# arpitbansal297/Cold-Diffusion-Models

Measured on AMD Instinct MI355X. Metric: unet_train_imgs_per_sec, higher is better.
Workload: dtype f32 storage/accumulate; dense-conv GEMM operands bf16x3; 1 GPU; CelebA-128 denoising cold diffusion (BASELINE config 3): Unet(dim=64,(1,2,4,8),ch=3) @128x128, T=200, optimizer step = 2 micro-batches x 32 img (one fused forward / backward pass over all of them: same draws, same gradient sum) + Adam + EMA/10; per_gpu_batch=32, gradient_accumulate_every=2, parallelism=single

## Files before the change

cold-diffusion-models_amd/csrc/k_conv_rowhalo.hip:

```cpp
#include "cdf_conv_sp.h"

template <int W, int BN, int NS = 3, int NCH = 2, int BM = 256>
__global__ void __launch_bounds__(512, 1) conv_igemm_rowhalo_stream_kernel(SpxArgs a) {
    constexpr int WM = BM / 64, WN = 8 / WM, NW = 8, BK = 32, RE = CDF_SP_RE, MT = BM / WM / 32, NB = 3;
    static_assert(BM == 256 && WM * WN == 8 && MT == 2, "8 waves (4 x 2) of 64-row tiles");
    static_assert(NCH % 2 == 0, "an even number of tap-row groups per tile returns the pipeline to row buffer 0");
    using L = RowHaloLayout<W, BN, BM>;
    using Segs = typename L::Segs;
    constexpr int EROWS = L::EROWS, CP = L::CP;
    constexpr int TH = L::TH, HW2 = L::HW2, RH = L::RH;
    constexpr int TAG = Segs::PER_WAVE;
    constexpr int NT = BN / WN / 32;
    constexpr int SB = BN / 16 / NW;
    static_assert(SB * NW * 16 == BN || BN == 64, "B tile must split into 16-row segments");
    constexpr int SBI = BN == 64 ? 1 : SB;
    constexpr int PLANE_A = L::PLANE_A, PLANE_B = L::PLANE_B;
    CDF_DYN_SMEM(smem_raw);
    unsigned short* smem = (unsigned short*)smem_raw;
    float* const cs = (float*)(smem + L::OFF_CS);

    const int tid = threadIdx.x, lane = tid & 63, wave = __builtin_amdgcn_readfirstlane(tid >> 6);
    const int wm = wave / WN, wn = wave % WN;
    const int M = a.B * a.QH * a.QW;
    const int tiles_n = (a.Cout + BN - 1) / BN, tiles_m = M / BM, ntiles = tiles_m * tiles_n;
    const CdfPhase& ph = a.ph[0];
    const int tpi = a.H / TH;

    const int srow = cdf_dma_row(lane), q8 = cdf_dma_col(lane);
    int a_seg[TAG], a_ry[TAG], a_x[TAG];
#pragma unroll
    for (int q = 0; q < TAG; ++q) {
        const int g = a_seg[q] = Segs::seg(wave, q);
        const int r = g * 16 + srow;
        a_ry[q] = r < RH ? r / HW2 : -(1 << 20);
        a_x[q] = r - (r / HW2) * HW2 - 1;
    }
    auto fetch_a = [&](int img, int y0, int c, int dy, int buf) {
        unsigned short* base = smem + L::a_off(buf);
#pragma unroll
        for (int q = 0; q < TAG; ++q) {
            const int y = y0 + a_ry[q] + dy;
            const bool ok = img >= 0 && (unsigned)y < (unsigned)a.H && (unsigned)a_x[q] < (unsigned)W;
            const size_t off = ((size_t)(((ok ? img : 0) * a.H + (ok ? y : 0)) * W + (ok ? a_x[q] : 0))) * (unsigned)a.ldx + (unsigned)(c * BK + q8);
            unsigned short* seg = base + a_seg[q] * 16 * RE;
            CDF_GLDS16_K(ok ? a.x_hi + off : a.zero, seg);
            if constexpr (NS == 3) CDF_GLDS16_K(ok ? a.x_lo + off : a.zero, seg + PLANE_A);
        }
    };
    auto fetch_b = [&](int tile_n, int c, int wi, int stage) {
        unsigned short* st = smem + L::b_off(stage);
#pragma unroll
        for (int p = 0; p < SBI; ++p) {
            const int seg = BN == 64 ? (wave & 3) : wave * SB + p;
            const size_t woff = cdf_w_off(wi, a.Cout, cdf_w_row(tile_n * BN + seg * 16 + srow, a.Cout), a.ldk, c * BK + q8);
            CDF_GLDS16_K(a.w_hi + woff, st + seg * 16 * RE);
            if constexpr (NS == 3) CDF_GLDS16_K(a.w_lo + woff, st + PLANE_B + seg * 16 * RE);
        }
    };
    constexpr int NPL = NS == 3 ? 2 : 1;
    constexpr int PB = NPL * SBI, PAG = NPL * TAG;

    const int half = lane >> 5, l31 = lane & 31;
    int row0[MT];
#pragma unroll
    for (int i = 0; i < MT; ++i) {
        const int pix = wm * (BM / WM) + i * 32 + l31;
        const int py = pix / W, px = pix - py * W;
        row0[i] = py * HW2 + px + 1;
    }
    const bool late = a.dephase != 0 && wave >= NW / 2;

    auto tile_pos = [&](int v, int& img, int& y0, int& tn, int& tm) {
        if (v < ntiles) {
            const int tile = cdf_xcd_order(v, ntiles);
            tm = tile / tiles_n;
            tn = tile - tm * tiles_n;
            img = tm / tpi;
            y0 = (tm - img * tpi) * TH;
        } else {
            img = -1; y0 = 0; tn = 0; tm = 0;
        }
    };
    int img, y0, tile_n, tile_m;
    int v = blockIdx.x;
    tile_pos(v, img, y0, tile_n, tile_m);
    const bool fast_epi = cdf_epi_tile_ok<BM, BN>(a, M) && cdf_epi_family_ok(a.epi, NS == 1);
    fetch_a(img, y0, 0, ph.dy[0], 0);
    fetch_b(tile_n, 0, ph.wi[0], 0);
    fetch_b(tile_n, 0, ph.wi[1], 1);
    CDF_WAIT_DMA_LEAVE(PB);
    CDF_LDS_BARRIER();

    while (img >= 0) {
        int img_n, y0_n, tile_n_n, tile_m_n;
        tile_pos(v + gridDim.x, img_n, y0_n, tile_n_n, tile_m_n);
        f32x16_t acc[MT][NT];
        cdf_acc_zero(acc);
        bf16x8_v ah[2][MT], al[2][MT], bh[2][NT], bl[2][NT];
        if (late) cdf_frag_zero(ah, al, bh, bl);
        auto mma_frags = [&]() { cdf_mma_tile<NS, MT, NT>(acc, ah, al, bh, bl); };
        int row0t[MT], l31t = l31;
#pragma unroll
        for (int i = 0; i < MT; ++i) row0t[i] = row0[i];
#ifndef CDF_EMU
#pragma unroll
        for (int i = 0; i < MT; ++i) asm volatile("" : "+v"(row0t[i]));
        asm volatile("" : "+v"(l31t));
#endif
        const int swbt = (l31t >> 2) & 3;
#pragma unroll
        for (int g = 0; g < 3; ++g) {
#pragma unroll
            for (int c = 0; c < NCH; ++c) {
#pragma unroll
                for (int i3 = 0; i3 < 3; ++i3) {
                    const int t = 3 * g + i3;
                    const int step = (g * NCH + c) * 3 + i3;
                    const int par = (g * NCH + c) & 1, rd = step % NB;
                    {
                        const int s2 = step + 2, gc2 = (s2 / 3) % (3 * NCH);
                        const bool over = s2 >= 9 * NCH;
                        const int g2 = gc2 / NCH, c2 = gc2 - g2 * NCH;
                        fetch_b(over ? tile_n_n : tile_n, c2, ph.wi[3 * g2 + s2 % 3], s2 % NB);
                    }
                    if (i3 == 0) {
                        const bool lastc = c + 1 == NCH, over = lastc && g == 2;
                        const int nc = lastc ? 0 : c + 1, ng = over ? 0 : (lastc ? g + 1 : g);
                        fetch_a(over ? img_n : img, over ? y0_n : y0, nc, ph.dy[3 * ng], par ^ 1);
                    }
                    int sa_e = L::a_off(par), sb_e = L::b_off(rd);
#ifndef CDF_EMU
                    asm volatile("" : "+s"(sa_e), "+s"(sb_e));
#endif
                    const unsigned short* sa = smem + sa_e;
                    const unsigned short* sb = smem + sb_e;
                    const int dx = ph.dx[t];
                    auto read_frags = [&]() {
#pragma unroll
                        for (int ks = 0; ks < 2; ++ks) {
                            cdf_read_frags_halo<NS, PLANE_A>(ah[ks], al[ks], sa, ks, half, row0t, dx);
                            cdf_read_frags<NS, PLANE_B>(bh[ks], bl[ks], sb, ks, half, wn * (BN / WN) + l31t, swbt);
                        }
                    };
                    cdf_dephased_step(late, read_frags, mma_frags);
                    if (i3 <= 1)
                        CDF_WAIT_DMA_LEAVE(PB + PAG);
                    else
                        CDF_WAIT_DMA_LEAVE(PB);
                    CDF_LDS_BARRIER();
                }
            }
        }
        if (late) mma_frags();
        auto dump = [&](int hp) {
            if ((wm * 64) / EROWS == hp) {
                int base = (wm * 64 - hp * EROWS + 4 * half) * CP + wn * (BN / WN) + l31;
#ifndef CDF_EMU
                asm volatile("" : "+v"(base));
#endif
                cdf_acc_stage(cs + base, CP, 0, 0, acc, 0, 0);
            }
        };
        if (fast_epi) {
            const long long trow = (long long)tile_m * BM;
            cdf_epi_dispatch<NS == 1>(a.epi, [&](auto spec) {
                using E = cdf_epi_fast<BN, EROWS, 512, decltype(spec)>;
                f32x4_t q[E::NR], bs[2];
                cdf_epi_load_bias<BN, 512>(a, bs, trow, tile_n * BN, tid);
                E::load(a, q, trow, tile_n * BN, tid);
                dump(0);
                CDF_LDS_BARRIER();
                E::template finish<true>(a, q, bs, cs, trow, tile_n * BN, tid, trow + EROWS);
                CDF_LDS_BARRIER();
                dump(1);
                CDF_LDS_BARRIER();
                E::template finish<false>(a, q, bs, cs, trow + EROWS, tile_n * BN, tid);
                CDF_LDS_BARRIER();
            });
        } else {
#pragma unroll 1
            for (int hp = 0; hp < 2; ++hp) {
                dump(hp);
                CDF_LDS_BARRIER();
                cdf_epilogue_rows<BN, EROWS, 512>(a, ph, a.y, cs, tile_m * BM + hp * EROWS, tile_n * BN, M, tid, [](int p) { return p; });
                CDF_LDS_BARRIER();
            }
        }
        img = img_n; y0 = y0_n; tile_n = tile_n_n; tile_m = tile_m_n;
        v += gridDim.x;
    }
    CDF_WAIT_DMA_LEAVE(0);
}

template <int NS, int W, int BN>
static int launch_igemm_rowhalo_stream(const SpxArgs& a, int M, hipStream_t s, int reserve, CdfPlan* plan) {
    using L = RowHaloLayout<W, BN>;
    const int tiles = (M / 256) * cdf_cdiv(a.Cout, BN);
#ifdef CDF_EMU
    int ncu = cdf_num_cus() - reserve;
    if (ncu < 1) ncu = 1;
#else
    int ncu = cdf_num_cus() - (reserve + 7) / 8 * 8;
    if (ncu < 8) ncu = 8;
#endif
    const int grid = tiles < ncu ? tiles : ncu;
    if (plan) return cdf_plan_set(plan, CDF_FORM_ROWHALO, 256, BN, a.Cin == 64 ? 2 : 4, 1, W, tiles, grid);
    if (a.Cin == 64)
        CDF_LAUNCH_LDS((conv_igemm_rowhalo_stream_kernel<W, BN, NS, 2>), dim3(grid), dim3(512), L::bytes, s, a);
    else
        CDF_LAUNCH_LDS((conv_igemm_rowhalo_stream_kernel<W, BN, NS, 4>), dim3(grid), dim3(512), L::bytes, s, a);
    return cdf_check_launch("conv_igemm_rowhalo_stream");
}


template <int NS>
static int launch_rowhalo_ns(int W, bool n64, const SpxArgs& a, int M, hipStream_t s, int reserve, CdfPlan* plan) {
#define CDF_ROWHALO_CASE(WW) \
    if (W == WW) return n64 ? launch_igemm_rowhalo_stream<NS, WW, 64>(a, M, s, reserve, plan) : launch_igemm_rowhalo_stream<NS, WW, 128>(a, M, s, reserve, plan);
    CDF_ROWHALO_CASE(128)
#ifdef CDF_EMU
    CDF_ROWHALO_CASE(64) CDF_ROWHALO_CASE(32) CDF_ROWHALO_CASE(16)
#endif
#undef CDF_ROWHALO_CASE
    return CDF_E_UNSUPPORTED;
}

int cdf_launch_igemm_rowhalo(int ns, int W, bool n64, const SpxArgs& a, int M, hipStream_t s, int reserve, CdfPlan* plan) {
    return ns == 3 ? launch_rowhalo_ns<3>(W, n64, a, M, s, reserve, plan) : launch_rowhalo_ns<1>(W, n64, a, M, s, reserve, plan);
}
```

cold-diffusion-models_amd/csrc/k_conv_spx.hip:

```cpp
#include "cdf_conv_sp.h"

template <int BM, int BN, int WM, int WN, int NSTAGE, int OCC = 512 / (64 * WM * WN), int NS = 3>
__global__ void __launch_bounds__(64 * WM * WN, OCC) conv_igemm_spx_kernel(SpxArgs a) {
    constexpr int BK = 32, RE = CDF_SP_RE, NW = WM * WN;
    constexpr int MT = BM / WM / 32, NT = BN / WN / 32;
    constexpr int SA = BM / 16 / NW, SB = BN / 16 / NW;
    static_assert(SA >= 1 && SB >= 1 && SA * NW * 16 == BM && SB * NW * 16 == BN, "tile must split into 16-row segments per wave");
    using L = SpxLayout<BM, BN, NSTAGE>;
    constexpr int PLANE_A = L::PLANE_A, PLANE_B = L::PLANE_B, STAGE = L::STAGE;
    CDF_DYN_SMEM(smem_raw);
    unsigned short* smem = (unsigned short*)smem_raw;

    const int tid = threadIdx.x, lane = tid & 63, wave = __builtin_amdgcn_readfirstlane(tid >> 6);
    const int wm = wave / WN, wn = wave % WN;
    const int M = a.B * a.QH * a.QW;
    const int tiles_n = (a.Cout + BN - 1) / BN, tiles_m = (M + BM - 1) / BM;
    const int tile = cdf_xcd_order(blockIdx.x, tiles_m * tiles_n);
    const int tile_m = tile / tiles_n, tile_n = tile - tile_m * tiles_n;
    const CdfPhase& ph = a.ph[blockIdx.y];

    const int srow = cdf_dma_row(lane), q8 = cdf_dma_col(lane);
    int a_iy0[SA], a_ix0[SA], b_row[SB];
    unsigned a_pix[SA];
#pragma unroll
    for (int p = 0; p < SA; ++p) {
        const int m = tile_m * BM + (wave * SA + p) * 16 + srow;
        if (m < M) {
            const int qx = m % a.QW, t2 = m / a.QW;
            a_iy0[p] = (t2 % a.QH) * a.is;
            a_ix0[p] = qx * a.is;
            a_pix[p] = (unsigned)(((t2 / a.QH) * a.H + a_iy0[p]) * a.W + a_ix0[p]);
        } else {
            a_iy0[p] = -(1 << 28);
            a_ix0[p] = 0;
            a_pix[p] = 0;
        }
    }
#pragma unroll
    for (int p = 0; p < SB; ++p) {
        b_row[p] = cdf_w_row(tile_n * BN + (wave * SB + p) * 16 + srow, a.Cout);
    }
    const int nchunks = (a.Cin + BK - 1) / BK;
    const int ntaps_blk = a.ksplit > 1 ? ph.ntaps / a.ksplit : ph.ntaps;
    const int tap_lo = a.ksplit > 1 ? (int)blockIdx.z * ntaps_blk : 0;
    const int niter = ntaps_blk * nchunks;

    int* tap_lds = (int*)(smem + L::OFF_TAPS);
    if (tid <= CDF_MAX_TAPS) {
        int src = tid + tap_lo;
        if (src > CDF_MAX_TAPS) src = CDF_MAX_TAPS;
        if (a.taprot && tid < 9) {
            const int slot = tid / 3, kx = tid - 3 * slot;
#pragma unroll
            for (int g = 0; g < 3; ++g) {
                const int r = (tile_m + (int)ph.dy[3 * g]) % 3;
                if ((r < 0 ? r + 3 : r) == slot) src = 3 * g + kx;
            }
        }
        tap_lds[tid] = src < ph.ntaps ? (ph.dy[src] & 0xFF) | ((ph.dx[src] & 0xFF) << 8) | ((ph.wi[src] & 0xFF) << 16) : 0;
    }
    CDF_LDS_BARRIER();

    const unsigned short* pa_hi[SA];
    const unsigned short* pa_lo[SA];
    const unsigned short* pb_hi[SB];
    const unsigned short* pb_lo[SB];
    int a_inc[SA];
    const bool ragged = (a.Cin & (BK - 1)) != 0;
    auto retap = [&](int tap) {
        const int tc = tap_lds[tap];
        const int dy = (int)(signed char)(tc & 0xFF), dx = (int)(signed char)((tc >> 8) & 0xFF), wi = (tc >> 16) & 0xFF;
        const int tap_pix = dy * a.W + dx;
#pragma unroll
        for (int p = 0; p < SA; ++p) {
            const unsigned iy = (unsigned)(a_iy0[p] + dy), ix = (unsigned)(a_ix0[p] + dx);
            const bool ok = iy < (unsigned)a.H && ix < (unsigned)a.W && q8 < a.Cin;
            const size_t off = (size_t)(a_pix[p] + (unsigned)tap_pix) * (unsigned)a.ldx + (unsigned)q8;
            pa_hi[p] = ok ? a.x_hi + off : a.zero;
            pa_lo[p] = ok ? a.x_lo + off : a.zero;
            a_inc[p] = ok ? BK : 0;
        }
#pragma unroll
        for (int p = 0; p < SB; ++p) {
            const size_t woff = cdf_w_off(wi, a.Cout, b_row[p], a.ldk, q8);
            pb_hi[p] = a.w_hi + woff;
            pb_lo[p] = a.w_lo + woff;
        }
    };
    int tap = 0, c0 = 0, issued = 0;
    retap(0);
    auto fetch = [&](int buf) {
        unsigned short* st = smem + buf * STAGE;
        const bool cok = !ragged || (c0 + q8) < a.Cin;
#pragma unroll
        for (int p = 0; p < SA; ++p) {
            unsigned short* seg = st + (wave * SA + p) * 16 * RE;
            CDF_GLDS16(cok ? pa_hi[p] : a.zero, seg);
            if constexpr (NS == 3) CDF_GLDS16(cok ? pa_lo[p] : a.zero, seg + PLANE_A);
        }
#pragma unroll
        for (int p = 0; p < SB; ++p) {
            unsigned short* seg = st + L::OFF_B + (wave * SB + p) * 16 * RE;
            CDF_GLDS16(pb_hi[p], seg);
            if constexpr (NS == 3) CDF_GLDS16(pb_lo[p], seg + PLANE_B);
        }
        const bool more = issued + 1 < niter;
        issued += more ? 1 : 0;
        if (more) {
            c0 += BK;
            if (c0 >= a.Cin) {
                c0 = 0;
                ++tap;
                retap(tap);
            } else {
#pragma unroll
                for (int p = 0; p < SA; ++p) {
                    pa_hi[p] += a_inc[p];
                    pa_lo[p] += a_inc[p];
                }
#pragma unroll
                for (int p = 0; p < SB; ++p) {
                    pb_hi[p] += BK;
                    pb_lo[p] += BK;
                }
            }
        }
    };

    f32x16_t acc[MT][NT];
    cdf_acc_zero(acc);

    const int half = lane >> 5, l31 = lane & 31;
    const int sw = (l31 >> 2) & 3;
    constexpr int PIECES = (NS == 3 ? 2 : 1) * (SA + SB);
    int fbuf = 0;
    if (niter > 0) {
#pragma unroll
        for (int d = 0; d < NSTAGE - 1; ++d) {
            fetch(fbuf);
            fbuf = fbuf + 1 == NSTAGE ? 0 : fbuf + 1;
        }
    }
    CDF_WAIT_DMA_LEAVE((NSTAGE - 2) * PIECES);
    CDF_LDS_BARRIER();
    int buf = 0;
    bf16x8_v ah[2][MT], al[2][MT], bh[2][NT], bl[2][NT];
    const bool late = a.dephase != 0 && NW == 8 && wave >= 4;
    if (late) cdf_frag_zero(ah, al, bh, bl);
    auto fetch_read = [&]() {
        fetch(fbuf);
        fbuf = fbuf + 1 == NSTAGE ? 0 : fbuf + 1;
        const unsigned short* sa = smem + buf * STAGE;
        const unsigned short* sb = sa + L::OFF_B;
        buf = buf + 1 == NSTAGE ? 0 : buf + 1;
#pragma unroll
        for (int ks = 0; ks < 2; ++ks) {
            cdf_read_frags<NS, PLANE_A>(ah[ks], al[ks], sa, ks, half, wm * (BM / WM) + l31, sw);
            cdf_read_frags<NS, PLANE_B>(bh[ks], bl[ks], sb, ks, half, wn * (BN / WN) + l31, sw);
        }
    };
    auto mma_frags = [&]() { cdf_mma_tile<NS, MT, NT>(acc, ah, al, bh, bl); };
    for (int it = 0; it < niter; ++it) {
        cdf_dephased_step(late, fetch_read, mma_frags);
        CDF_WAIT_DMA_LEAVE((NSTAGE - 2) * PIECES);
        CDF_LDS_BARRIER();
    }
    if (late) mma_frags();
    CDF_WAIT_DMA_LEAVE(0);
    CDF_LDS_BARRIER();

    if (a.ksplit > 1) {
        RawEpiArgs r;
        r.Cout = a.Cout; r.vec = (a.Cout & 3) == 0 ? 1 : 0; r.os = 1; r.QH = 1; r.QW = 1; r.OH = 1; r.OW = 1; r.ldy = a.ks_ld;
        r.ldp = r.ldm = r.ldr = r.ld_sbias = r.ld_ys = 0; r.act = 0; r.mul_mode = 0; r.accumulate = 0;
        r.bias = nullptr; r.sbias = nullptr; r.pre = nullptr; r.mul = nullptr; r.res = nullptr; r.ys_hi = nullptr; r.ys_lo = nullptr; r.io_bf = 0;
        float* cs = (float*)smem_raw;
        cdf_acc_stage(cs, BN + 8, wm * (BM / WM), wn * (BN / WN), acc, half, l31);
        __syncthreads();
        cdf_epilogue_rows<BN, BM, 64 * WM * WN>(r, ph, a.ks_ws + (size_t)blockIdx.z * M * a.ks_ld, cs, tile_m * BM, tile_n * BN, M, tid,
                                                [](int p) { return p; });
        return;
    }
    cdf_sp_epilogue<BM, BN, WM, WN, NS == 1>(a, ph, acc, (float*)smem_raw, tile_m, tile_n, M, tid);
}

template <int BN>
__global__ void __launch_bounds__(256) conv_splitk_finish_kernel(SpxArgs a) {
    constexpr int BM = 16, CP = BN + 8;
    __shared__ __attribute__((aligned(16))) float cs[BM * CP];
    const int tid = threadIdx.x;
    const int M = a.B * a.QH * a.QW;
    const int tiles_n = (a.Cout + BN - 1) / BN;
    const int tile_m = blockIdx.x / tiles_n, tile_n = blockIdx.x - tile_m * tiles_n;
    constexpr int V = BN / 4;
    const size_t zs = (size_t)M * a.ks_ld;
    for (int e = tid; e < BM * V; e += 256) {
        const int r = e / V, c4 = (e - r * V) * 4;
        const int m = tile_m * BM + r, n = tile_n * BN + c4;
        const bool ok = m < M && n < a.ks_ld;
        const float* p = a.ks_ws + (ok ? (size_t)m * a.ks_ld + n : 0);
        float4 v[CDF_MAX_TAPS];
#pragma unroll
        for (int z = 0; z < CDF_MAX_TAPS; ++z) v[z] = *(const float4*)(p + (z < a.ksplit ? z : 0) * zs);
        float4 sum = make_float4(0.f, 0.f, 0.f, 0.f);
#pragma unroll
        for (int z = 0; z < CDF_MAX_TAPS; ++z)
            if (z < a.ksplit) { sum.x += v[z].x; sum.y += v[z].y; sum.z += v[z].z; sum.w += v[z].w; }
        *(float4*)(cs + r * CP + c4) = ok ? sum : make_float4(0.f, 0.f, 0.f, 0.f);
    }
    __syncthreads();
    cdf_epilogue_rows<BN, BM, 256>(a, a.ph[0], a.y, cs, tile_m * BM, tile_n * BN, M, tid, [](int p) { return p; });
}

extern "C" int cdf_gemm_tuning_default(cdf_gemm_tuning* t) {
    CDF_REQUIRE(t, "cdf_gemm_tuning_default: null pointer");
    *t = kTuneDefault;
    return 0;
}

template <int NS, int BM, int BN, int WM, int WN, int NSTAGE, int OCC = 512 / (64 * WM * WN)>
static int launch_igemm_spx(const SpxArgs& a, int M, hipStream_t s, CdfPlan* plan) {
    using L = SpxLayout<BM, BN, NSTAGE>;
    const int tiles = cdf_cdiv(M, BM) * cdf_cdiv(a.Cout, BN);
    if (plan) return cdf_plan_set(plan, CDF_FORM_SPX, BM, BN, NSTAGE, a.ksplit > 1 ? a.ksplit : 1, 0, tiles, (long long)tiles * a.nphase * (a.ksplit > 1 ? a.ksplit : 1));
    CDF_LAUNCH_LDS((conv_igemm_spx_kernel<BM, BN, WM, WN, NSTAGE, OCC, NS>), dim3(tiles, a.nphase, a.ksplit > 1 ? a.ksplit : 1), dim3(64 * WM * WN), L::bytes, s, a);
    if (a.ksplit > 1) {
        const int ftiles = cdf_cdiv(M, 16) * cdf_cdiv(a.Cout, BN);
        if (BN == 64) CDF_LAUNCH((conv_splitk_finish_kernel<64>), dim3(ftiles), dim3(256), 0, s, a);
        else CDF_LAUNCH((conv_splitk_finish_kernel<128>), dim3(ftiles), dim3(256), 0, s, a);
    }
    return cdf_check_launch("conv_igemm_spx");
}

static int spx_ksplit(int M, int Cout, int nphase, int ntaps, const cdf_gemm_tuning& T) {
    if (!T.splitk || !T.deep || nphase != 1 || (ntaps != 9 && ntaps != 16)) return 1;
    const bool n64 = Cout <= 64;
    const long long tiles128 = (long long)cdf_cdiv(M, 128) * cdf_cdiv(Cout, n64 ? 64 : 128);
    const long long tiles64 = (long long)cdf_cdiv(M, 64) * cdf_cdiv(Cout, n64 ? 64 : 128);
    if (tiles128 >= 384 || tiles64 > 128) return 1;
    for (int ks = 2; ks <= ntaps; ++ks)
        if (ntaps % ks == 0 && tiles64 * ks >= 192) return ks;
    return ntaps;
}
extern "C" int cdf_conv_gemm_bf16x_ksplit(int M, int Cout, int nphase, int ntaps, const cdf_gemm_tuning* tune) { return spx_ksplit(M, Cout, nphase, ntaps, *cdf_tune(tune)); }

template <int NS>
static int dispatch_gemm_bf16x(SpxArgs& a, long long ks_ws_floats, const cdf_gemm_tuning& T, hipStream_t s, int* bm_out = nullptr, CdfPlan* plan = nullptr) {
    const int B = a.B, H = a.H, W = a.W, Cin = a.Cin, Cout = a.Cout, QH = a.QH, QW = a.QW, os = a.os, is = a.is, nphase = a.nphase;
    const int M = B * QH * QW;
    const bool n64 = T.tile_bn ? T.tile_bn == 64 : Cout <= 64;
    const long long tiles128 = (long long)cdf_cdiv(M, 128) * cdf_cdiv(Cout, n64 ? 64 : 128) * nphase;
    bool m64 = tiles128 < 384;
    bool m256 = !n64 && tiles128 >= 1024 && T.max_bm != 128;
    if (T.tile_bm) { m64 = T.tile_bm == 64; m256 = T.tile_bm == 256 && !n64; }
    bool is3x3 = nphase == 1 && is == 1 && os == 1 && a.ph[0].ntaps == 9 && a.ph[0].oy == 0 && a.ph[0].ox == 0;
    if (is3x3) {
        int seen = 0;
        for (int g = 0; g < 3; ++g) {
            const int dy = a.ph[0].dy[3 * g];
            is3x3 = is3x3 && a.ph[0].dy[3 * g + 1] == dy && a.ph[0].dy[3 * g + 2] == dy && dy >= -1 && dy <= 1;
            seen |= 1 << (dy + 1);
        }
        is3x3 = is3x3 && seen == 7;
    }
    const bool rot_ok = is3x3;
    const int bm = m256 ? 256 : (m64 ? 64 : 128);
    a.taprot = rot_ok && QW == bm;
    a.dephase = T.dephase;
    if (T.halo && is3x3 && !T.tile_bm && QW == W && QH == H && Cin % 32 == 0 && Cin >= 64 && M % 128 == 0) {
        const bool n64_in = n64;
        int dxs = 0;
        for (int t = 0; t < 9; ++t) dxs |= 1 << (a.ph[0].dx[t] + 1);
        const bool dx_ok = dxs == 7;
        const bool n64 = n64_in || (T.small_n64 && !T.tile_bn && Cout > 64 && Cout % 64 == 0 && (long long)(M / 128) * cdf_cdiv(Cout, 128) < 176);
        const long long tiles = (long long)(M / 128) * cdf_cdiv(Cout, n64 ? 64 : 128);
        if (dx_ok && M % 256 == 0 && (T.rowhalo_stream & 1) && (Cin == 64 || Cin == 128) &&
            ((T.halo & 64) || ((T.halo & 32) && W == 128 && !n64 && (long long)(M / 256) * cdf_cdiv(Cout, 128) >= 256))) {
            if ((W == 128 || W == 64 || W == 32 || W == 16) && H % (256 / W) == 0) {
                const int rc = cdf_launch_igemm_rowhalo(NS, W, n64, a, M, s, T.resident_reserve, plan);
                if (rc != CDF_E_UNSUPPORTED) return rc;
            }
        }
        if (dx_ok && tiles >= (T.halo_min_tiles > 0 ? T.halo_min_tiles : 1)) {
            if ((W == 128 || W == 64 || W == 32 || W == 16) && (T.halo & (W / 16)) && H % (128 / W) == 0 && (W < 128 || n64 || (T.halo & 16))) {
                const bool bm256 = (W <= 64 || n64) && T.halo_bm != 128 && H % (256 / W) == 0 && M % 256 == 0 &&
                                   (T.halo_bm == 256 || (long long)(M / 256) * cdf_cdiv(Cout, n64 ? 64 : 128) >= 256);
                if (bm_out) *bm_out = bm256 ? 256 : 128;
                return cdf_launch_igemm_halo(NS, W, n64, bm256 ? 256 : 128, a, M, s, plan);
            }
        }
    }
    if (bm_out) *bm_out = bm;
    if (m256) return launch_igemm_spx<NS, 256, 128, 4, 2, 3>(a, M, s, plan);
    const long long tiles64 = (long long)cdf_cdiv(M, 64) * cdf_cdiv(Cout, n64 ? 64 : 128) * nphase;
    if (m64 && tiles64 <= 256 && T.deep) {
        const int ks = spx_ksplit(M, Cout, nphase, a.ph[0].ntaps, T);
        if (ks > 1 && a.ks_ws && ks_ws_floats >= (long long)ks * M * ((Cout + 3) / 4 * 4)) {
            a.ksplit = ks;
            a.ks_ld = (Cout + 3) / 4 * 4;
            a.taprot = 0;
        } else {
            a.ksplit = 1;
        }
        if (n64) return launch_igemm_spx<NS, 64, 64, 2, 2, 6, 1>(a, M, s, plan);
        return launch_igemm_spx<NS, 64, 128, 2, 2, 6, 1>(a, M, s, plan);
    }
    if (n64) return m64 ? launch_igemm_spx<NS, 64, 64, 2, 2, 2>(a, M, s, plan) : launch_igemm_spx<NS, 128, 64, 2, 2, 2>(a, M, s, plan);
    if (m64) return launch_igemm_spx<NS, 64, 128, 2, 2, 2>(a, M, s, plan);
    return launch_igemm_spx<NS, 128, 128, 2, 2, 2>(a, M, s, plan);
}

extern "C" int cdf_conv_gemm_bf16x_io(const void* x_hi, const void* x_lo, int ldx, const void* zero, const void* w_hi, const void* w_lo,
                                      int ldk, float* y, int ldy, int B, int H, int W, int Cin, int OH, int OW, int Cout, int QH, int QW,
                                      int os, int is, int nphase, const int* phase_desc, const float* bias, const float* sbias,
                                      int ld_sbias, const void* res, int ldr, void* pre, int ldp, const void* mul, int ldm, int act,
                                      int mul_mode, int accumulate, int io_bf16, void* y_hi, void* y_lo, int ld_ys, float* ws,
                                      long long ws_floats, const cdf_gemm_tuning* tune, void* stream);

extern "C" int cdf_conv_gemm_bf16x(const void* x_hi, const void* x_lo, int ldx, const void* zero, const void* w_hi, const void* w_lo,
                                   int ldk, float* y, int ldy, int B, int H, int W, int Cin, int OH, int OW, int Cout, int QH, int QW,
                                   int os, int is, int nphase, const int* phase_desc, const float* bias, const float* sbias,
                                   int ld_sbias, const float* res, int ldr, float* pre, int ldp, const float* mul, int ldm, int act,
                                   int mul_mode, int accumulate, void* y_hi, void* y_lo, int ld_ys, float* ws, long long ws_floats,
                                   const cdf_gemm_tuning* tune, void* stream) {
    return cdf_conv_gemm_bf16x_io(x_hi, x_lo, ldx, zero, w_hi, w_lo, ldk, y, ldy, B, H, W, Cin, OH, OW, Cout, QH, QW, os, is, nphase, phase_desc,
                                  bias, sbias, ld_sbias, res, ldr, pre, ldp, mul, ldm, act, mul_mode, accumulate, 0, y_hi, y_lo, ld_ys, ws,
                                  ws_floats, tune, stream);
}

extern "C" int cdf_conv_gemm_bf16x_io(const void* x_hi, const void* x_lo, int ldx, const void* zero, const void* w_hi, const void* w_lo,
                                      int ldk, float* y, int ldy, int B, int H, int W, int Cin, int OH, int OW, int Cout, int QH, int QW,
                                      int os, int is, int nphase, const int* phase_desc, const float* bias, const float* sbias,
                                      int ld_sbias, const void* res_, int ldr, void* pre_, int ldp, const void* mul_, int ldm, int act,
                                      int mul_mode, int accumulate, int io_bf16, void* y_hi, void* y_lo, int ld_ys, float* ws,
                                      long long ws_floats, const cdf_gemm_tuning* tune, void* stream) {
    const float* res = (const float*)res_;
    float* pre = (float*)pre_;
    const float* mul = (const float*)mul_;
    CDF_REQUIRE((io_bf16 & ~15) == 0, "cdf_conv_gemm_bf16x_io: io_bf16 has unknown bits (%d)", io_bf16);
    CDF_REQUIRE(!(io_bf16 & CDF_IO_PRE_GRAD) || (pre_ && (act == 1 || act == 2)), "cdf_conv_gemm_bf16x_io: CDF_IO_PRE_GRAD needs a pre tensor and act = GELU / SiLU");
    CDF_REQUIRE(x_hi && zero && w_hi && (y || (y_hi && !accumulate)), "cdf_conv_gemm_bf16x: null pointer");
    CDF_TUNE_CHECK(tune, "cdf_conv_gemm_bf16x");
    CDF_REQUIRE(!ws || (((uintptr_t)ws) & 15) == 0, "cdf_conv_gemm_bf16x: the split-K workspace must be 16-byte aligned");
    CDF_REQUIRE((x_lo != nullptr) == (w_lo != nullptr), "cdf_conv_gemm_bf16x: pass both lo planes (split precision, 3 MFMAs per product) or neither (single-pass bf16)");
    CDF_REQUIRE((!y_hi && !y_lo) || (y_hi && ld_ys % 4 == 0 && ld_ys >= Cout && Cout % 4 == 0 && ((((uintptr_t)y_hi) | ((uintptr_t)y_lo)) & 7) == 0),
                "cdf_conv_gemm_bf16x: output planes need Cout %% 4 == 0, ld_ys %% 4 == 0, 8-byte alignment (y_lo optional: hi-only planes)");
    CDF_REQUIRE(((((uintptr_t)x_hi) | ((uintptr_t)x_lo) | ((uintptr_t)zero) | ((uintptr_t)w_hi) | ((uintptr_t)w_lo)) & 15) == 0, "cdf_conv_gemm_bf16x: operands must be 16B aligned");
    CDF_REQUIRE(ldx % 8 == 0 && Cin % 8 == 0 && ldx >= Cin && ldk % 32 == 0 && ldk >= Cin, "cdf_conv_gemm_bf16x: Cin and pitches must be multiples of 8 (ldk of 32)");
    CDF_REQUIRE(nphase >= 1 && nphase <= 4 && phase_desc && (!y || ldy >= Cout), "cdf_conv_gemm_bf16x: bad geometry");
    CDF_REQUIRE(!mul_mode || mul, "cdf_conv_gemm_bf16x: mul_mode without mul tensor");
    SpxArgs a;
    a.x_hi = (const unsigned short*)x_hi; a.x_lo = (const unsigned short*)x_lo; a.zero = (const unsigned short*)zero;
    a.w_hi = (const unsigned short*)w_hi; a.w_lo = (const unsigned short*)w_lo; a.ldx = ldx; a.ldk = ldk;
    cdf_fill_gemm_common(a, y, ldy, bias, sbias, ld_sbias, res, ldr, pre, ldp, mul, ldm, B, H, W, Cin, OH, OW, Cout, QH, QW, os, is, nphase, act, mul_mode,
                         accumulate, y_hi, y_lo, ld_ys, io_bf16);
    cdf_clear_epi(a);
    if (cdf_tune(tune)->epilogue) a.epi = cdf_epi_select(a);
    CDF_REQUIRE(!y_hi || a.vec, "cdf_conv_gemm_bf16x: split output planes need the vectorised epilogue (aligned pointers, pitches %% 4)");
    CDF_REQUIRE(!(io_bf16 & 7) || a.vec, "cdf_conv_gemm_bf16x_io: bf16 epilogue operands need the vectorised epilogue (16-byte-aligned pointers, pitches %% 4, Cout %% 4)");
    int rc = cdf_fill_phases(a.ph, nphase, phase_desc, "cdf_conv_gemm_bf16x");
    if (rc) return rc;
    a.ksplit = 1; a.ks_ws = ws; a.ks_ld = 0;
    return x_lo ? dispatch_gemm_bf16x<3>(a, ws ? ws_floats : 0, *cdf_tune(tune), CDF_S)
                : dispatch_gemm_bf16x<1>(a, ws ? ws_floats : 0, *cdf_tune(tune), CDF_S);
}


extern "C" int cdf_conv_gemm_bf16x_lnbwd_ok(int B, int H, int W, int Cin, int Cout, int nphase, int ntaps) {
    const long long M = (long long)B * H * W;
    return (Cout == 64 || Cout == 128) && nphase == 1 && ntaps == 9 && M % 256 == 0 && M < (1ll << 31) && Cin % 32 == 0 && Cin >= 64;
}
static cdf_gemm_tuning lnbwd_tuning(const cdf_gemm_tuning* tune) {
    cdf_gemm_tuning T = *cdf_tune(tune);
    T.rowhalo_stream = 0; T.small_n64 = 0; T.tile_bn = 0; T.splitk = 0;
    return T;
}

extern "C" int cdf_conv_gemm_bf16x_form(int B, int H, int W, int Cin, int Cout, int QH, int QW, int os, int is, int nphase, const int* phase_desc,
                                        int ns, long long ws_floats, int lnbwd, const cdf_gemm_tuning* tune, int* tiles_grid) {
    CDF_REQUIRE(phase_desc && nphase >= 1 && nphase <= 4 && (ns == 1 || ns == 3) && B >= 1, "cdf_conv_gemm_bf16x_form: bad arguments");
    CDF_TUNE_CHECK(tune, "cdf_conv_gemm_bf16x_form");
    CDF_REQUIRE(!lnbwd || cdf_conv_gemm_bf16x_lnbwd_ok(B, H, W, Cin, Cout, nphase, phase_desc[2]), "cdf_conv_gemm_bf16x_form: not a geometry of cdf_conv_gemm_bf16x_lnbwd");
    SpxArgs a = {};
    cdf_fill_gemm_common(a, nullptr, 0, nullptr, nullptr, 0, nullptr, 0, nullptr, 0, nullptr, 0, B, H, W, Cin, 0, 0, Cout, QH, QW, os, is, nphase, 0, 0, 0, nullptr, nullptr, 0, 0);
    int rc = cdf_fill_phases(a.ph, nphase, phase_desc, "cdf_conv_gemm_bf16x_form");
    if (rc) return rc;
    static float ws_token;
    a.ksplit = 1; a.ks_ws = (ws_floats > 0 && !lnbwd) ? &ws_token : nullptr; a.ks_ld = 0;
    const cdf_gemm_tuning T = lnbwd ? lnbwd_tuning(tune) : *cdf_tune(tune);
    CdfPlan plan = {0, 0, 0};
    rc = ns == 3 ? dispatch_gemm_bf16x<3>(a, a.ks_ws ? ws_floats : 0, T, nullptr, nullptr, &plan)
                 : dispatch_gemm_bf16x<1>(a, a.ks_ws ? ws_floats : 0, T, nullptr, nullptr, &plan);
    if (rc) return rc;
    if (tiles_grid) { tiles_grid[0] = plan.tiles; tiles_grid[1] = plan.grid; }
    return plan.code;
}

extern "C" int cdf_conv_gemm_bf16x_lnbwd(const void* x_hi, const void* x_lo, int ldx, const void* zero, const void* w_hi, const void* w_lo, int ldk,
                                         int B, int H, int W, int Cin, int Cout, const int* phase_desc, const float* ln_x, int ld_lnx,
                                         const float* ln_mean, const float* ln_rstd, const float* ln_g, float* dh, int lddh, float* dg, float* db,
                                         float* part, const cdf_gemm_tuning* tune, void* stream) {
    CDF_REQUIRE(x_hi && zero && w_hi && phase_desc && ln_x && ln_mean && ln_rstd && ln_g && dh && dg && db && part, "cdf_conv_gemm_bf16x_lnbwd: null pointer");
    CDF_TUNE_CHECK(tune, "cdf_conv_gemm_bf16x_lnbwd");
    CDF_REQUIRE((x_lo != nullptr) == (w_lo != nullptr), "cdf_conv_gemm_bf16x_lnbwd: pass both lo planes or neither");
    CDF_REQUIRE(cdf_conv_gemm_bf16x_lnbwd_ok(B, H, W, Cin, Cout, 1, phase_desc[2]), "cdf_conv_gemm_bf16x_lnbwd: needs a 3 x 3 stride-1 layer with 64 or 128 output channels, B*H*W %% 256 == 0");
    CDF_REQUIRE(((((uintptr_t)x_hi) | ((uintptr_t)x_lo) | ((uintptr_t)zero) | ((uintptr_t)w_hi) | ((uintptr_t)w_lo) | ((uintptr_t)ln_x) | ((uintptr_t)ln_g) | ((uintptr_t)dh)) & 15) == 0 &&
                ldx % 8 == 0 && ldx >= Cin && ldk % 32 == 0 && ldk >= Cin && ld_lnx % 4 == 0 && ld_lnx >= Cout && lddh % 4 == 0 && lddh >= Cout,
                "cdf_conv_gemm_bf16x_lnbwd: alignment / pitches");
    SpxArgs a;
    a.x_hi = (const unsigned short*)x_hi; a.x_lo = (const unsigned short*)x_lo; a.zero = (const unsigned short*)zero;
    a.w_hi = (const unsigned short*)w_hi; a.w_lo = (const unsigned short*)w_lo; a.ldx = ldx; a.ldk = ldk;
    cdf_fill_gemm_common(a, dh, lddh, ln_g, nullptr, 0, nullptr, 0, nullptr, 0, nullptr, 0, B, H, W, Cin, H, W, Cout, H, W, 1, 1, 1, 0, 0, 0, nullptr, nullptr, 0, 0);
    a.vec = 1;
    a.epi = CDF_EPI_LNBWD;
    a.ln_x = ln_x; a.ln_mean = ln_mean; a.ln_rstd = ln_rstd; a.ln_part = part; a.ld_lnx = ld_lnx;
    int rc = cdf_fill_phases(a.ph, 1, phase_desc, "cdf_conv_gemm_bf16x_lnbwd");
    if (rc) return rc;
    a.ksplit = 1; a.ks_ws = nullptr; a.ks_ld = 0;
    const cdf_gemm_tuning T = lnbwd_tuning(tune);
    int bm = 0;
    rc = x_lo ? dispatch_gemm_bf16x<3>(a, 0, T, CDF_S, &bm) : dispatch_gemm_bf16x<1>(a, 0, T, CDF_S, &bm);
    if (rc) return rc;
    CDF_REQUIRE(bm == 64 || bm == 128 || bm == 256, "cdf_conv_gemm_bf16x_lnbwd: the dispatcher reported no row tile");
    return cdf_norm_param_reduce(part, (int)((long long)B * H * W / bm), Cout, dg, db, 1, stream);
}
```

Measured before the change: 1310 img/s.

## Use 16x16 MFMA tiles for bf16x3 conv kernels on selected configurations

```diff
diff --git a/cold-diffusion-models_amd/csrc/k_conv_rowhalo.hip b/cold-diffusion-models_amd/csrc/k_conv_rowhalo.hip
--- a/cold-diffusion-models_amd/csrc/k_conv_rowhalo.hip
+++ b/cold-diffusion-models_amd/csrc/k_conv_rowhalo.hip
@@ -1,8 +1,14 @@
 #include "cdf_conv_sp.h"
+
+constexpr int cdf_rowhalo_mfma(int W, int BN, int NS) {
+    (void)W; (void)BN;
+    return NS == 3 ? 16 : 32;
+}
 
 template <int W, int BN, int NS = 3, int NCH = 2, int BM = 256>
 __global__ void __launch_bounds__(512, 1) conv_igemm_rowhalo_stream_kernel(SpxArgs a) {
     constexpr int WM = BM / 64, WN = 8 / WM, NW = 8, BK = 32, RE = CDF_SP_RE, MT = BM / WM / 32, NB = 3;
+    constexpr int MF = cdf_rowhalo_mfma(W, BN, NS);
     static_assert(BM == 256 && WM * WN == 8 && MT == 2, "8 waves (4 x 2) of 64-row tiles");
     static_assert(NCH % 2 == 0, "an even number of tap-row groups per tile returns the pipeline to row buffer 0");
     using L = RowHaloLayout<W, BN, BM>;
@@ -26,7 +32,7 @@
     const CdfPhase& ph = a.ph[0];
     const int tpi = a.H / TH;
 
-    const int srow = cdf_dma_row(lane), q8 = cdf_dma_col(lane);
+    const int srow = cdf_dma_row(lane), q8 = cdf_dma_col<MF>(lane);
     int a_seg[TAG], a_ry[TAG], a_x[TAG];
 #pragma unroll
     for (int q = 0; q < TAG; ++q) {
@@ -61,13 +67,17 @@
     constexpr int PB = NPL * SBI, PAG = NPL * TAG;
 
     const int half = lane >> 5, l31 = lane & 31;
-    int row0[MT];
-#pragma unroll
-    for (int i = 0; i < MT; ++i) {
-        const int pix = wm * (BM / WM) + i * 32 + l31;
-        const int py = pix / W, px = pix - py * W;
-        row0[i] = py * HW2 + px + 1;
-    }
+    constexpr int NF = MF == 16 ? 2 : 1;
+    const int lrow = MF == 16 ? lane & 15 : l31, kblk = MF == 16 ? lane >> 4 : half;
+    int row0[NF][MT];
+#pragma unroll
+    for (int f = 0; f < NF; ++f)
+#pragma unroll
+        for (int i = 0; i < MT; ++i) {
+            const int pix = wm * (BM / WM) + i * 32 + f * 16 + lrow;
+            const int py = pix / W, px = pix - py * W;
+            row0[f][i] = py * HW2 + px + 1;
+        }
     const bool late = a.dephase != 0 && wave >= NW / 2;
 
     auto tile_pos = [&](int v, int& img, int& y0, int& tn, int& tm) {
@@ -94,20 +104,24 @@
     while (img >= 0) {
         int img_n, y0_n, tile_n_n, tile_m_n;
         tile_pos(v + gridDim.x, img_n, y0_n, tile_n_n, tile_m_n);
-        f32x16_t acc[MT][NT];
+        typename cdf_acc_of<MF>::type acc[MT][NT];
         cdf_acc_zero(acc);
         bf16x8_v ah[2][MT], al[2][MT], bh[2][NT], bl[2][NT];
         if (late) cdf_frag_zero(ah, al, bh, bl);
         auto mma_frags = [&]() { cdf_mma_tile<NS, MT, NT>(acc, ah, al, bh, bl); };
-        int row0t[MT], l31t = l31;
-#pragma unroll
-        for (int i = 0; i < MT; ++i) row0t[i] = row0[i];
+        int row0t[NF][MT], lrowt = lrow;
+#pragma unroll
+        for (int f = 0; f < NF; ++f)
+#pragma unroll
+            for (int i = 0; i < MT; ++i) row0t[f][i] = row0[f][i];
 #ifndef CDF_EMU
 #pragma unroll
-        for (int i = 0; i < MT; ++i) asm volatile("" : "+v"(row0t[i]));
-        asm volatile("" : "+v"(l31t));
-#endif
-        const int swbt = (l31t >> 2) & 3;
+        for (int f = 0; f < NF; ++f)
+#pragma unroll
+            for (int i = 0; i < MT; ++i) asm volatile("" : "+v"(row0t[f][i]));
+        asm volatile("" : "+v"(lrowt));
+#endif
+        const int swbt = cdf_swz<MF>(lrowt);
 #pragma unroll
         for (int g = 0; g < 3; ++g) {
 #pragma unroll
@@ -138,8 +152,8 @@
                     auto read_frags = [&]() {
 #pragma unroll
                         for (int ks = 0; ks < 2; ++ks) {
-                            cdf_read_frags_halo<NS, PLANE_A>(ah[ks], al[ks], sa, ks, half, row0t, dx);
-                            cdf_read_frags<NS, PLANE_B>(bh[ks], bl[ks], sb, ks, half, wn * (BN / WN) + l31t, swbt);
+                            cdf_read_frags_halo<NS, PLANE_A, MT, MF>(ah[ks], al[ks], sa, ks, kblk, row0t[MF == 16 ? ks : 0], dx);
+                            cdf_read_frags<NS, PLANE_B, NT, MF>(bh[ks], bl[ks], sb, ks, kblk, wn * (BN / WN) + (MF == 16 ? 16 * ks : 0) + lrowt, swbt);
                         }
                     };
                     cdf_dephased_step(late, read_frags, mma_frags);
@@ -154,7 +168,7 @@
         if (late) mma_frags();
         auto dump = [&](int hp) {
             if ((wm * 64) / EROWS == hp) {
-                int base = (wm * 64 - hp * EROWS + 4 * half) * CP + wn * (BN / WN) + l31;
+                int base = (wm * 64 - hp * EROWS + 4 * kblk) * CP + wn * (BN / WN) + lrow;
 #ifndef CDF_EMU
                 asm volatile("" : "+v"(base));
 #endif
diff --git a/cold-diffusion-models_amd/csrc/k_conv_spx.hip b/cold-diffusion-models_amd/csrc/k_conv_spx.hip
--- a/cold-diffusion-models_amd/csrc/k_conv_spx.hip
+++ b/cold-diffusion-models_amd/csrc/k_conv_spx.hip
@@ -1,8 +1,15 @@
 #include "cdf_conv_sp.h"
+
+constexpr int cdf_spx_mfma(int BM, int BN, int WM, int WN, int NSTAGE, int NS) {
+    (void)WM; (void)WN;
+    if (NS == 3) return BN == 128 && NSTAGE <= 3 ? 16 : 32;
+    return BM == 128 && BN == 128 ? 16 : 32;
+}
 
 template <int BM, int BN, int WM, int WN, int NSTAGE, int OCC = 512 / (64 * WM * WN), int NS = 3>
 __global__ void __launch_bounds__(64 * WM * WN, OCC) conv_igemm_spx_kernel(SpxArgs a) {
     constexpr int BK = 32, RE = CDF_SP_RE, NW = WM * WN;
+    constexpr int MF = cdf_spx_mfma(BM, BN, WM, WN, NSTAGE, NS);
     constexpr int MT = BM / WM / 32, NT = BN / WN / 32;
     constexpr int SA = BM / 16 / NW, SB = BN / 16 / NW;
     static_assert(SA >= 1 && SB >= 1 && SA * NW * 16 == BM && SB * NW * 16 == BN, "tile must split into 16-row segments per wave");
@@ -19,7 +26,7 @@
     const int tile_m = tile / tiles_n, tile_n = tile - tile_m * tiles_n;
     const CdfPhase& ph = a.ph[blockIdx.y];
 
-    const int srow = cdf_dma_row(lane), q8 = cdf_dma_col(lane);
+    const int srow = cdf_dma_row(lane), q8 = cdf_dma_col<MF>(lane);
     int a_iy0[SA], a_ix0[SA], b_row[SB];
     unsigned a_pix[SA];
 #pragma unroll
@@ -127,11 +134,12 @@
         }
     };
 
-    f32x16_t acc[MT][NT];
+    typename cdf_acc_of<MF>::type acc[MT][NT];
     cdf_acc_zero(acc);
 
     const int half = lane >> 5, l31 = lane & 31;
-    const int sw = (l31 >> 2) & 3;
+    const int lrow = MF == 16 ? lane & 15 : l31, kblk = MF == 16 ? lane >> 4 : half;
+    const int sw = cdf_swz<MF>(lrow);
     constexpr int PIECES = (NS == 3 ? 2 : 1) * (SA + SB);
     int fbuf = 0;
     if (niter > 0) {
@@ -155,8 +163,8 @@
         buf = buf + 1 == NSTAGE ? 0 : buf + 1;
 #pragma unroll
         for (int ks = 0; ks < 2; ++ks) {
-            cdf_read_frags<NS, PLANE_A>(ah[ks], al[ks], sa, ks, half, wm * (BM / WM) + l31, sw);
-            cdf_read_frags<NS, PLANE_B>(bh[ks], bl[ks], sb, ks, half, wn * (BN / WN) + l31, sw);
+            cdf_read_frags<NS, PLANE_A, MT, MF>(ah[ks], al[ks], sa, ks, kblk, wm * (BM / WM) + (MF == 16 ? 16 * ks : 0) + lrow, sw);
+            cdf_read_frags<NS, PLANE_B, NT, MF>(bh[ks], bl[ks], sb, ks, kblk, wn * (BN / WN) + (MF == 16 ? 16 * ks : 0) + lrow, sw);
         }
     };
     auto mma_frags = [&]() { cdf_mma_tile<NS, MT, NT>(acc, ah, al, bh, bl); };
```

New measurement: 1318 img/s (median of 6 runs). No clear change (+0.6%).
